# lukedan/libfluid

Hardware: AMD Instinct MI355X
Metric: particle_steps_per_sec (higher is better)
Workload: dtype f32

## Files before the change

libfluid_amd/csrc/particles.hip:

```cpp
#include <math.h>

#include <algorithm>
#include <utility>

#include "common.h"
#include "pcg.h"

namespace {

__device__ inline bool solid_or_outside(const GridDims &g, const uint8_t *solid, int x, int y, int z) {
	if (!in_grid(g, x, y, z)) return true;
	return solid[blocked_index(g, x, y, z)] != 0;
}

__device__ inline void collide(const GridDims &g, const uint8_t *solid, double from[3], double to[3], double skin) {
	for (int bounce = 0; bounce < 3; ++bounce) {
		bool hit = false;
		double diff[3], inv[3], t[3];
		int cur[3], last[3], adv[3];
#pragma unroll
		for (int d = 0; d < 3; ++d) {
			cur[d] = (int)floor(from[d]);
			last[d] = (int)floor(to[d]);
			diff[d] = to[d] - from[d];
// ... 60 lines not shown
		if (cp < skin && ci == 0) x += skin - cp;
		if (cp > skin_max && ci + 1 >= n[d]) x += skin_max - cp;
		to[d] = x;
	}
}

__device__ inline void cell_of_key(const GridDims &g, uint32_t key, int c[3]) {
	int tile = (int)(key >> 9), l = (int)(key & 511), tx, ty, tz;
	tile_coords(g, tile, tx, ty, tz);
	c[0] = tx * 8 + (l & 7); c[1] = ty * 8 + ((l >> 3) & 7); c[2] = tz * 8 + (l >> 6);
}
__device__ inline void split_position(double p, int n, int &cell, float &t) {
	double m = p < 0.0 ? 0.0 : p;
	int c = m >= (double)n ? n - 1 : (int)m;
	double td = p - (double)c;
	float tf = (float)td;
	if (!(tf > 0.0f)) tf = 0.0f;
	if (td < 1.0 && tf >= 1.0f) tf = 0.99999994f;
	if (tf > 1.0f) tf = 1.0f;
	cell = c;
	t = tf;
}

#ifndef CORR_PARTS
#define CORR_PARTS 2
#endif
#define CORR_THREADS 512
#define CORR_THREADS_BIG 1024
#ifndef CORR_STAGE_DEPTH
#define CORR_STAGE_DEPTH 4
#endif
#define CORR_BIG_SLICES 4

struct MoveParams {
	double dt_over_h;
	double skin;
	double corr;
	double inv_re2;
	float *c_home;
	size_t c_home_stride;
	int collide;
};

__global__ void __launch_bounds__(256) k_tile_has_solid(const uint8_t *solid, int nt, uint8_t *tile_solid) {
	for (int t = blockIdx.x; t < nt; t += gridDim.x) {
		const uint8_t *c = solid + (size_t)t * LFA_TILE_CELLS;
		const int any = __syncthreads_or((c[threadIdx.x] | c[threadIdx.x + 256]) != 0);
		if (threadIdx.x == 0) tile_solid[t] = (uint8_t)(any ? 1 : 0);
	}
}
__global__ void k_tile_clear(GridDims g, const uint8_t *tile_solid, uint8_t *tile_clear) {
	const int t = blockIdx.x * blockDim.x + threadIdx.x;
	if (t >= g.nt) return;
	int tx, ty, tz;
	tile_coords(g, t, tx, ty, tz);
	int any = 0;
	for (int dz = -1; dz <= 1; ++dz)
		for (int dy = -1; dy <= 1; ++dy)
			for (int dx = -1; dx <= 1; ++dx) {
				const int x = tx + dx, y = ty + dy, z = tz + dz;
				if ((unsigned)x < (unsigned)g.ntx && (unsigned)y < (unsigned)g.nty && (unsigned)z < (unsigned)g.ntz)
					any |= tile_solid[x + g.ntx * (y + g.nty * z)];
			}
	tile_clear[t] = (uint8_t)(any ? 0 : 1);
}

template <bool COERCE>
__device__ inline uint32_t advect_one(size_t i, const ParticleSoA &p, const GridDims &g, const uint8_t *solid, const MoveParams &mp,
                                      const uint8_t *coerce_map, const float *src_vel, const uint8_t *tile_clear) {
	const uint32_t key = p.key[i];
	if (key == 0xFFFFFFFFu) return key;
	int c[3];
	cell_of_key(g, key, c);
	const int nn[3] = {g.nx, g.ny, g.nz};
	float vel[3] = {p.v[0][i], p.v[1][i], p.v[2][i]};
	if (COERCE) {
		const uint32_t src = coerce_map[key];
		if (src) {
#pragma unroll
			for (int d = 0; d < 3; ++d) {
				vel[d] = src_vel[3 * (src - 1) + d];
				p.v[d][i] = vel[d];
			}
			if (mp.c_home) {
				const size_t j = p.id[i];
#pragma unroll
				for (int k = 0; k < 9; ++k) mp.c_home[k * mp.c_home_stride + j] = 0.0f;
			} else {
#pragma unroll
				for (int k = 0; k < 9; ++k) p.c[k][i] = 0.0f;
			}
		}
	}
	double from[3], to[3];
#pragma unroll
	for (int d = 0; d < 3; ++d) {
		from[d] = (double)c[d] + (double)p.t[d][i];
		double x = from[d] + (double)vel[d] * mp.dt_over_h;
		const double lo = mp.skin, hi = (double)nn[d] - mp.skin;
		to[d] = x < lo ? lo : (hi < x ? hi : x);
	}
	const bool open_water = (tile_clear[key >> 9] & 1) && fabs(to[0] - from[0]) < 7.0 && fabs(to[1] - from[1]) < 7.0 &&
	                        fabs(to[2] - from[2]) < 7.0;
	if (!open_water && mp.collide) collide(g, solid, from, to, mp.skin);
	int nc[3];
	float nt[3];
#pragma unroll
	for (int d = 0; d < 3; ++d) split_position(to[d], nn[d], nc[d], nt[d]);
	const uint32_t new_key = blocked_index(g, nc[0], nc[1], nc[2]);
	p.key[i] = new_key;
#pragma unroll
	for (int d = 0; d < 3; ++d) p.t[d][i] = nt[d];
	return new_key;
}

template <bool COERCE>
__global__ void __launch_bounds__(256)
k_advect_collide(size_t n, ParticleSoA p, GridDims g, const uint8_t *solid, MoveParams mp, const uint8_t *coerce_map,
                 const float *src_vel, const uint8_t *tile_clear) {
	const size_t i = (size_t)blockIdx.x * blockDim.x + threadIdx.x;
	if (i < n) advect_one<COERCE>(i, p, g, solid, mp, coerce_map, src_vel, tile_clear);
}

#define AC_CHUNKS 8
template <bool COERCE>
__global__ void __launch_bounds__(256)
k_advect_collide_count(size_t n, ParticleSoA p, GridDims g, const uint8_t *solid, MoveParams mp, const uint8_t *coerce_map,
                       const float *src_vel, const uint8_t *tile_clear, uint32_t *tile_count, uint32_t *rank) {
	const int lane = threadIdx.x & 63;
	const size_t wave = ((size_t)blockIdx.x * blockDim.x + threadIdx.x) >> 6;
	const size_t i0 = wave * (64 * AC_CHUNKS) + lane;
	uint32_t tile[AC_CHUNKS], my_rank[AC_CHUNKS];
#pragma unroll
	for (int c = 0; c < AC_CHUNKS; ++c) {
		const size_t i = i0 + 64 * c;
		const uint32_t k = i < n ? advect_one<COERCE>(i, p, g, solid, mp, coerce_map, src_vel, tile_clear) : 0xFFFFFFFFu;
		tile[c] = k != 0xFFFFFFFFu ? k >> 9 : 0xFFFFFFFFu;
	}
	lfa_wave_tile_ranks(tile, tile_count, my_rank);
#pragma unroll
	for (int c = 0; c < AC_CHUNKS; ++c) {
		const size_t i = i0 + 64 * c;
		if (tile[c] != 0xFFFFFFFFu) rank[i] = my_rank[c];
	}
}

__device__ inline float hash_unit(uint32_t a, uint32_t b, uint32_t k) {
	uint32_t x = a * 0x9E3779B1u ^ (b + 0x7F4A7C15u) * 0x85EBCA77u ^ k * 0xC2B2AE3Du;
	x ^= x >> 15; x *= 0x2C1B3C6Du; x ^= x >> 12; x *= 0x297A2D39u; x ^= x >> 15;
	return (float)(x >> 8) * (2.0f / 16777216.0f) - 1.0f;
}

#define FT 11
#define FT3 (FT * FT * FT)
#define FT_STRIDE (FT3 + 1)
#define FT_INV 1.375f
#define FT_PL ((FT + CORR_PARTS - 1) / CORR_PARTS)
#define FB 13
#define FBZ (FT_PL + 2)
#define FB_N (FB * FB * FBZ)
#define FB_ROWS (FB * FBZ)
#define FINE_CAP 5632
#define FINE_CAP_BIG 12288
#define FIDX_THREADS 512
#define FIDX_CNT 1536
#define FIDX_STAGE 4608

__device__ inline int fine_coord(int l, float t) {
	const int f = (int)(((float)l + t) * FT_INV);
	return f < FT - 1 ? f : FT - 1;
}
__device__ inline float4 fine_record(int lx, int ly, int lz, float t0, float t1, float t2, uint32_t index) {
	const uint32_t b0 = (__float_as_uint(t0) & 0x3FFFFFFFu) | ((uint32_t)(lx & 3) << 30);
	const uint32_t b1 = (__float_as_uint(t1) & 0x3FFFFFFFu) | ((uint32_t)(lx >> 2) << 31) | ((uint32_t)(ly & 1) << 30);
	const uint32_t b2 = (__float_as_uint(t2) & 0x3FFFFFFFu) | ((uint32_t)(lz & 1) << 31);
	return make_float4(__uint_as_float(b0), __uint_as_float(b1), __uint_as_float(b2), __uint_as_float(index));
}
__device__ inline void fine_decode_at(const float4 &r, int y0, int z0, float t[3], int l[3]) {
	const uint32_t b0 = __float_as_uint(r.x), b1 = __float_as_uint(r.y), b2 = __float_as_uint(r.z);
	t[0] = __uint_as_float(b0 & 0x3FFFFFFFu); t[1] = __uint_as_float(b1 & 0x3FFFFFFFu); t[2] = __uint_as_float(b2 & 0x3FFFFFFFu);
	l[0] = (int)(b0 >> 30) | ((int)(b1 >> 31) << 2);
	l[1] = y0 + ((y0 ^ (int)(b1 >> 30)) & 1);
	l[2] = z0 + ((z0 ^ (int)(b2 >> 31)) & 1);
}
__device__ inline void fine_decode(const float4 &r, int fy, int fz, float t[3], int l[3]) {
	fine_decode_at(r, (8 * fy) / FT, (8 * fz) / FT, t, l);
}

__global__ void __launch_bounds__(FIDX_THREADS)
k_build_fine_index(const int *ptiles, int n_ptiles, const uint32_t *key, const float *t0, const float *t1, const float *t2,
                   const uint32_t *tile_start, const uint32_t *tile_count, uint32_t *fine_start, float4 *spos, uint32_t *key_copy) {
	__shared__ uint32_t cnt[FIDX_CNT];
	__shared__ uint32_t wsum[FIDX_THREADS / 64];
	__shared__ float4 stage[FIDX_STAGE];
	static_assert(FIDX_CNT % FIDX_THREADS == 0 && FIDX_STAGE % FIDX_THREADS == 0, "index kernel sizing");
	constexpr int PER = FIDX_CNT / FIDX_THREADS;
	auto fine_of = [&](uint32_t i, int l[3], float t[3]) -> int {
		const uint32_t k = key[i];
		l[0] = (int)(k & 7); l[1] = (int)((k >> 3) & 7); l[2] = (int)((k >> 6) & 7);
		t[0] = t0[i]; t[1] = t1[i]; t[2] = t2[i];
		return fine_coord(l[0], t[0]) + FT * (fine_coord(l[1], t[1]) + FT * fine_coord(l[2], t[2]));
	};
	constexpr int RPT = FIDX_STAGE / FIDX_THREADS;
	for (int slot = blockIdx.x; slot < n_ptiles; slot += gridDim.x) {
		const int tile = ptiles[slot];
		const uint32_t b = tile_start[tile], e = b + tile_count[tile];
		const bool staged = e - b <= FIDX_STAGE;
#pragma unroll
		for (int k = 0; k < PER; ++k) cnt[threadIdx.x + FIDX_THREADS * k] = 0;
		__syncthreads();
		uint32_t rf[RPT];
		float r0[RPT], r1[RPT], r2[RPT];
		if (staged) {
#pragma unroll
			for (int r = 0; r < RPT; ++r) {
				const uint32_t i = b + threadIdx.x + FIDX_THREADS * r;
				rf[r] = 0xFFFFFFFFu;
				if (i < e) {
					int l[3];
					float t[3];
					const int f = fine_of(i, l, t);
					rf[r] = ((uint32_t)f << 9) | (uint32_t)(l[0] | (l[1] << 3) | (l[2] << 6));
					r0[r] = t[0]; r1[r] = t[1]; r2[r] = t[2];
					atomicAdd(&cnt[f], 1u);
				}
			}
		} else {
			for (uint32_t i = b + threadIdx.x; i < e; i += FIDX_THREADS) {
				int l[3];
				float t[3];
				atomicAdd(&cnt[fine_of(i, l, t)], 1u);
			}
		}
		__syncthreads();
		uint32_t c[PER], incl = 0;
#pragma unroll
		for (int k = 0; k < PER; ++k) {
			c[k] = cnt[PER * threadIdx.x + k];
			incl += c[k];
		}
		const uint32_t sum = incl;
		const int lane = threadIdx.x & 63, wid = threadIdx.x >> 6;
#pragma unroll
		for (int o = 1; o < 64; o <<= 1) {
			uint32_t t = __shfl_up(incl, o, 64);
			if (lane >= o) incl += t;
		}
		if (lane == 63) wsum[wid] = incl;
		__syncthreads();
		uint32_t ex = b + incl - sum;
		for (int w = 0; w < wid; ++w) ex += wsum[w];
		__syncthreads();
#pragma unroll
		for (int k = 0; k < PER; ++k) {
			const int f = PER * threadIdx.x + k;
			cnt[f] = ex;
			if (f <= FT3) fine_start[(size_t)tile * FT_STRIDE + f] = ex;
			ex += c[k];
		}
		__syncthreads();
		if (staged) {
#pragma unroll
			for (int r = 0; r < RPT; ++r)
				if (rf[r] != 0xFFFFFFFFu) {
					const uint32_t at = atomicAdd(&cnt[rf[r] >> 9], 1u);
					stage[at - b] = fine_record((int)(rf[r] & 7), (int)((rf[r] >> 3) & 7), (int)((rf[r] >> 6) & 7), r0[r], r1[r], r2[r],
					                            b + threadIdx.x + FIDX_THREADS * r);
				}
			if (key_copy) {
#pragma unroll
				for (int r = 0; r < RPT; ++r)
					if (rf[r] != 0xFFFFFFFFu) key_copy[b + threadIdx.x + FIDX_THREADS * r] = ((uint32_t)tile << 9) | (rf[r] & 511u);
			}
			__syncthreads();
			for (uint32_t k = threadIdx.x; k < e - b; k += FIDX_THREADS) spos[b + k] = stage[k];
		} else {
			for (uint32_t i = b + threadIdx.x; i < e; i += FIDX_THREADS) {
				int l[3];
				float t[3];
				const uint32_t at = atomicAdd(&cnt[fine_of(i, l, t)], 1u);
				spos[at] = fine_record(l[0], l[1], l[2], t[0], t[1], t[2], i);
				if (key_copy) key_copy[i] = key[i];
			}
		}
		__syncthreads();
	}
}

__device__ inline int fine_source(const GridDims &g, const uint32_t *tile_count, int tx, int ty, int tz, int gx, int gy, int gz, int &fx,
                                  int &fy, int &fz) {
	const int dx = gx < 0 ? -1 : (gx >= FT ? 1 : 0), dy = gy < 0 ? -1 : (gy >= FT ? 1 : 0), dz = gz < 0 ? -1 : (gz >= FT ? 1 : 0);
	fx = gx - FT * dx; fy = gy - FT * dy; fz = gz - FT * dz;
	const int x = tx + dx, y = ty + dy, z = tz + dz;
	if ((unsigned)x >= (unsigned)g.ntx || (unsigned)y >= (unsigned)g.nty || (unsigned)z >= (unsigned)g.ntz) return -1;
	const int tile = x + g.ntx * (y + g.nty * z);
	return tile_count[tile] ? tile : -1;
}

__device__ inline void correct_collide_record(size_t rk, const ParticleSoA &p, uint32_t *out_key, float *out_tx, float *out_ty, float *out_tz,
                                              const GridDims &g, const uint8_t *solid, const uint32_t *tile_count, const uint32_t *fine_start,
                                              const float4 *spos, const MoveParams &mp, const uint32_t *only_flagged, const int *tile_pslot,
                                              int p_off, const uint32_t *key_before) {
	const float4 me = spos[rk];
	const size_t i = __float_as_uint(me.w);
	const uint32_t key_i = key_before ? key_before[i] : p.key[i];
	if (key_i == 0xFFFFFFFFu) return;
	const int tile = (int)(key_i >> 9);
	const int l[3] = {(int)(key_i & 7), (int)((key_i >> 3) & 7), (int)((key_i >> 6) & 7)};
	const float t[3] = {__uint_as_float(__float_as_uint(me.x) & 0x3FFFFFFFu), __uint_as_float(__float_as_uint(me.y) & 0x3FFFFFFFu),
	                    __uint_as_float(__float_as_uint(me.z) & 0x3FFFFFFFu)};
	const int f[3] = {fine_coord(l[0], t[0]), fine_coord(l[1], t[1]), fine_coord(l[2], t[2])};
	if (only_flagged) {
		const int work = CORR_PARTS * (tile_pslot[tile] - p_off) + f[2] / FT_PL;
		if (!((only_flagged[1 + (work >> 5)] >> (work & 31)) & 1u)) return;
	}
	int tx, ty, tz;
	tile_coords(g, tile, tx, ty, tz);
	const int nn[3] = {g.nx, g.ny, g.nz};
	const float inv_re2 = (float)mp.inv_re2;
	double spring[3] = {0.0, 0.0, 0.0};
	for (int dz = -1; dz <= 1; ++dz)
		for (int dy = -1; dy <= 1; ++dy)
			for (int dx = -1; dx <= 1; ++dx) {
				int sf[3];
				const int src = fine_source(g, tile_count, tx, ty, tz, f[0] + dx, f[1] + dy, f[2] + dz, sf[0], sf[1], sf[2]);
				if (src < 0) continue;
				const uint32_t *fs = fine_start + (size_t)src * FT_STRIDE + (sf[0] + FT * (sf[1] + FT * sf[2]));
				const uint32_t kb = fs[0], ke = fs[1];
				int stx, sty, stz;
				tile_coords(g, src, stx, sty, stz);
				for (uint32_t k = kb; k < ke; ++k) {
					const float4 rec = spos[k];
					if (__float_as_uint(rec.w) == (uint32_t)i) continue;
					float nt[3];
					int nl[3];
					fine_decode(rec, sf[1], sf[2], nt, nl);
					const float ddx = ((float)(8 * (tx - stx) + l[0] - nl[0]) + t[0]) - nt[0];
					const float ddy = ((float)(8 * (ty - sty) + l[1] - nl[1]) + t[1]) - nt[1];
					const float ddz = ((float)(8 * (tz - stz) + l[2] - nl[2]) + t[2]) - nt[2];
					const float d2 = ddx * ddx + ddy * ddy + ddz * ddz;
					if (d2 < 1e-12f) {
						const uint32_t j = __float_as_uint(rec.w);
						spring[0] += hash_unit((uint32_t)i, j, 0); spring[1] += hash_unit((uint32_t)i, j, 1);
						spring[2] += hash_unit((uint32_t)i, j, 2);
					} else {
						const float kl = 1.0f - d2 * inv_re2;
						if (kl > 0.0f) {
							const float fr = kl * kl * kl * rsqrtf(d2);
							spring[0] += (double)(fr * ddx); spring[1] += (double)(fr * ddy); spring[2] += (double)(fr * ddz);
						}
					}
				}
			}
	const int c[3] = {8 * tx + l[0], 8 * ty + l[1], 8 * tz + l[2]};
	double from[3], to[3];
#pragma unroll
	for (int d = 0; d < 3; ++d) {
		from[d] = (double)c[d] + (double)t[d];
		double x = from[d] + spring[d] * mp.corr;
		to[d] = x < 0.0 ? 0.0 : ((double)nn[d] < x ? (double)nn[d] : x);
	}
	if (mp.collide) collide(g, solid, from, to, mp.skin);
	int nc[3];
	float ntt[3];
#pragma unroll
	for (int d = 0; d < 3; ++d) split_position(to[d], nn[d], nc[d], ntt[d]);
	out_key[i] = blocked_index(g, nc[0], nc[1], nc[2]);
	out_tx[i] = ntt[0]; out_ty[i] = ntt[1]; out_tz[i] = ntt[2];
}

__global__ void __launch_bounds__(256)
k_correct_collide(size_t n, ParticleSoA p, uint32_t *out_key, float *out_tx, float *out_ty, float *out_tz, GridDims g,
                   const uint8_t *solid, const uint32_t *tile_count, const uint32_t *fine_start, const float4 *spos, MoveParams mp,
                   const uint32_t *only_flagged, const int *tile_pslot, int p_off, const uint32_t *key_before) {
	if (only_flagged && only_flagged[0] == 0) return;
	for (size_t rk = (size_t)blockIdx.x * blockDim.x + threadIdx.x; rk < n; rk += (size_t)gridDim.x * blockDim.x)
		correct_collide_record(rk, p, out_key, out_tx, out_ty, out_tz, g, solid, tile_count, fine_start, spos, mp, only_flagged, tile_pslot,
		                       p_off, key_before);
}

#ifdef CORR_PROFILE
__device__ unsigned long long g_corr_prof[8];
#define CORR_STAMP(k)                                                                   \
	do {                                                                                \
		if (!ONLY && threadIdx.x == 0) {                                                \
			const unsigned long long now_ = wall_clock64();                             \
			atomicAdd(&g_corr_prof[k], now_ - stamp_);                                  \
			stamp_ = now_;                                                              \
		}                                                                               \
	} while (0)
#else
#define CORR_STAMP(k) do { } while (0)
#endif
template <int CAP, bool ONLY>
__global__ void __launch_bounds__(ONLY ? CORR_THREADS_BIG : CORR_THREADS, 4)
k_correct_fine(const int *ptiles, int n_ptiles, uint32_t *out_key, float *out_tx, float *out_ty, float *out_tz, GridDims g,
                const uint8_t *solid, const uint32_t *tile_count, const uint32_t *fine_start, const float4 *spos, MoveParams mp,
                uint32_t *overflow_tiles, const uint8_t *tile_clear, const uint32_t *only) {
	constexpr int T = ONLY ? CORR_THREADS_BIG : CORR_THREADS;
	constexpr int CNT = ((FB_N + 1 + T - 1) / T) * T;
	__shared__ float px[CAP], py[CAP], pz[CAP];
	__shared__ uint32_t fcnt[CNT];
	__shared__ uint16_t foff[FB_N + 1];
	__shared__ __attribute__((aligned(16))) uint32_t rowd[FB_ROWS * 8];
	constexpr uint32_t ROW_NOT_OWN = 0x80000000u;
	__shared__ uint32_t ownoff[FT * FT_PL + 1];
	__shared__ int srct[27];
	__shared__ uint32_t wsum[T / 64];
	uint16_t *own = (uint16_t *)fcnt;
	static_assert(CNT > FB_N && CNT % T == 0, "fcnt sizing");
	constexpr int PER = CNT / T;
	const int nn[3] = {g.nx, g.ny, g.nz};
	const int lane = threadIdx.x & 63, wid = threadIdx.x >> 6;
	if (ONLY && only[0] == 0) return;
	constexpr int SLICES = ONLY ? CORR_BIG_SLICES : 1;
	for (int item = blockIdx.x; item < SLICES * CORR_PARTS * n_ptiles; item += gridDim.x) {
		const int work = item / SLICES, slice = item % SLICES;
		if (ONLY && !((only[1 + (work >> 5)] >> (work & 31)) & 1u)) continue;
		const int tile = ptiles[work / CORR_PARTS], part = work % CORR_PARTS;
		int tx, ty, tz;
		tile_coords(g, tile, tx, ty, tz);
		const int own_lo = part * FT_PL, own_n = (own_lo + FT_PL <= FT ? FT_PL : FT - own_lo);
		const int gz0 = own_lo - 1;
		const int nzb = own_n + 2;
		const int nrows = FB * nzb, nown_rows = FT * (nzb - 2);
		const bool open_water = (tile_clear[tile] & 1) != 0;
		const bool lean = open_water && mp.collide && tx >= 1 && ty >= 1 && tz >= 1 && 8 * tx + 16 <= g.nx && 8 * ty + 16 <= g.ny &&
		                  8 * tz + 16 <= g.nz;
		__syncthreads();
#ifdef CORR_PROFILE
		unsigned long long stamp_ = wall_clock64();
		if (!ONLY && threadIdx.x == 0) atomicAdd(&g_corr_prof[7], 1ull);
#endif
		uint32_t tid = threadIdx.x;
		asm volatile("" : "+v"(tid));
		if (tid < 27) {
			int fx, fy, fz;
			srct[tid] = fine_source(g, tile_count, tx, ty, tz, FT * ((int)tid % 3 - 1), FT * (((int)tid / 3) % 3 - 1), FT * ((int)tid / 9 - 1), fx,
			                        fy, fz);
		}
		__syncthreads();
#pragma unroll
		for (int k = 0; k < PER; ++k) {
			const int f = (int)(k == PER - 1 ? tid : threadIdx.x) + T * k;
			uint32_t cnt = 0, src0 = 0;
			if (f < FB * nrows) {
				const int bx = f % FB, row = f / FB, by = row % FB, bz = row / FB;
				const int gx = bx - 1, gy = by - 1, gz = gz0 + bz;
				const int dx = gx < 0 ? 0 : (gx >= FT ? 2 : 1), dy = gy < 0 ? 0 : (gy >= FT ? 2 : 1), dz = gz < 0 ? 0 : (gz >= FT ? 2 : 1);
				const int src = srct[dx + 3 * dy + 9 * dz];
				if (src >= 0) {
					const uint32_t fid = (uint32_t)((gx - FT * (dx - 1)) + FT * ((gy - FT * (dy - 1)) + FT * (gz - FT * (dz - 1))));
					const uint32_t *fs = fine_start + ((uint32_t)src * FT_STRIDE + fid);
					src0 = fs[0];
					cnt = fs[1] - src0;
				}
				if (bx <= 1 || bx == FB - 1) rowd[row * 8 + (bx <= 1 ? bx : 2)] = src0;
			}
			fcnt[f] = cnt;
		}
		__syncthreads();
		uint32_t c4[PER], sum = 0;
#pragma unroll
		for (int k = 0; k < PER; ++k) {
			c4[k] = fcnt[PER * threadIdx.x + k];
			sum += c4[k];
		}
		uint32_t incl = sum;
#pragma unroll
		for (int o = 1; o < 64; o <<= 1) {
			uint32_t t = __shfl_up(incl, o, 64);
			if (lane >= o) incl += t;
		}
		if (lane == 63) wsum[wid] = incl;
		__syncthreads();
		uint32_t woff = 0, total = 0;
		for (int w = 0; w < T / 64; ++w) {
			if (w < wid) woff += wsum[w];
			total += wsum[w];
		}
		if (total > (uint32_t)CAP) {
			if (threadIdx.x == 0 && slice == 0) {
				atomicOr(&overflow_tiles[1 + (work >> 5)], 1u << (work & 31));
				atomicAdd(&overflow_tiles[0], 1u);
			}
			continue;
		}
		{
			uint32_t ex = woff + incl - sum;
#pragma unroll
			for (int k = 0; k < PER; ++k) {
				const int f = PER * threadIdx.x + k;
				if (f <= FB_N) foff[f] = (uint16_t)ex;
				ex += c4[k];
			}
		}
		__syncthreads();
		uint32_t own_total = 0, own_first = 0;
		{
			uint32_t len = 0;
			if (tid < (unsigned)nown_rows) {
				const int row = (1 + (int)tid % FT) + FB * (1 + (int)tid / FT);
				len = (uint32_t)foff[row * FB + FB - 1] - (uint32_t)foff[row * FB + 1];
			}
			uint32_t in2 = len;
#pragma unroll
			for (int o = 1; o < 64; o <<= 1) {
				uint32_t t = __shfl_up(in2, o, 64);
				if (lane >= o) in2 += t;
			}
			if (lane == 63) wsum[wid] = in2;
			__syncthreads();
			uint32_t wo = 0;
			for (int w = 0; w < T / 64; ++w) {
				if (w < wid) wo += wsum[w];
				own_total += wsum[w];
			}
			own_first = wo + in2 - len;
			if (tid < (unsigned)nown_rows) ownoff[tid] = own_first;
			if (tid == 0) ownoff[nown_rows] = own_total;
		}
		const bool listed = own_total <= 2u * CNT;
		if (tid < (unsigned)nrows) {
			const int r = (int)tid, by = r % FB, bz = r / FB;
			const int gy = by - 1, gz = gz0 + bz;
			const int dy = gy < 0 ? -1 : (gy >= FT ? 1 : 0), dz = gz < 0 ? -1 : (gz >= FT ? 1 : 0);
			const int fy = gy - FT * dy, fz = gz - FT * dz;
			const uint32_t d0 = foff[r * FB], d1 = foff[r * FB + 1], d2 = foff[r * FB + FB - 1];
			uint32_t *rd = rowd + r * 8;
			rd[0] -= d0; rd[1] -= d1; rd[2] -= d2;
			rd[3] = d1 | (d2 << 16);
			rd[4] = (uint32_t)(8 * dy); rd[5] = (uint32_t)(8 * dz);
			rd[6] = (uint32_t)((8 * fy) / FT) | ((uint32_t)((8 * fz) / FT) << 8);
			if (!(listed && by >= 1 && by <= FT && bz >= 1 && bz <= nzb - 2)) rd[7] = ROW_NOT_OWN;
		}
		if (listed && tid < (unsigned)nown_rows) {
			const int row = (1 + (int)tid % FT) + FB * (1 + (int)tid / FT);
			rowd[row * 8 + 7] = own_first - (uint32_t)foff[row * FB + 1];
		}
		__syncthreads();
		CORR_STAMP(0);
		{
			static_assert(FB_ROWS <= 128, "two row starts per lane");
			const int rl = (int)(tid & 63u);
			const uint32_t rs_lo = rl < nrows ? (uint32_t)foff[rl * FB] : 0xFFFFFFFFu;
			const uint32_t rs_hi = rl + 64 < nrows ? (uint32_t)foff[(rl + 64) * FB] : 0xFFFFFFFFu;
			auto row_of = [&](uint32_t s) -> int {
				return (int)__popcll(__ballot(rs_lo <= s)) + (int)__popcll(__ballot(rs_hi <= s)) - 1;
			};
			auto locate = [&](uint32_t slot, int r_first, int r_last, uint32_t &src, int &rs) {
				int r = r_first;
				const int span = r_last - r_first;
				for (int step = span ? 1 << (31 - __builtin_clz(span)) : 0; step; step >>= 1) {
					const int c = r + step;
					if (c <= r_last && (uint32_t)foff[c * FB] <= slot) r = c;
				}
				const uint4 d = *(const uint4 *)(rowd + r * 8);
				const int seg = slot < (d.w & 0xFFFFu) ? 0 : (slot < (d.w >> 16) ? 1 : 2);
				src = (seg == 0 ? d.x : (seg == 1 ? d.y : d.z)) + slot;
				rs = r | (seg << 8);
			};
			auto put = [&](uint32_t slot, const float4 &rec, int rs) {
				const int r = rs & 255, seg = rs >> 8;
				const uint4 d = *(const uint4 *)(rowd + r * 8 + 4);
				float t[3];
				int l[3];
				fine_decode_at(rec, (int)(d.z & 255u), (int)(d.z >> 8), t, l);
				px[slot] = (float)(8 * (seg - 1) + l[0]) + t[0];
				py[slot] = (float)((int)d.x + l[1]) + t[1];
				pz[slot] = (float)((int)d.y + l[2]) + t[2];
				if (seg == 1 && d.w != ROW_NOT_OWN) own[d.w + slot] = (uint16_t)slot;
			};
			const uint32_t wave0 = (uint32_t)__builtin_amdgcn_readfirstlane((int)(threadIdx.x & ~63u));
			for (uint32_t w0 = wave0; w0 < total; w0 += CORR_STAGE_DEPTH * T) {
				uint32_t src[CORR_STAGE_DEPTH];
				int rs[CORR_STAGE_DEPTH];
				float4 rec[CORR_STAGE_DEPTH];
#pragma unroll
				for (int u = 0; u < CORR_STAGE_DEPTH; ++u) {
					const uint32_t wu = w0 + u * T, slot = wu + lane;
					src[u] = 0; rs[u] = 0;
					if (wu < total) {
						const uint32_t last = wu + 63 < total ? wu + 63 : total - 1;
						const int r_first = row_of(wu), r_last = row_of(last);
						if (slot < total) locate(slot, r_first, r_last, src[u], rs[u]);
					}
				}
#pragma unroll
				for (int u = 0; u < CORR_STAGE_DEPTH; ++u) rec[u] = spos[src[u]];
#pragma unroll
				for (int u = 0; u < CORR_STAGE_DEPTH; ++u) {
					const uint32_t slot = w0 + u * T + lane;
					if (slot < total) put(slot, rec[u], rs[u]);
				}
			}
		}
		__syncthreads();
		CORR_STAMP(1);
#ifdef CORR_PROFILE
		if (!ONLY && threadIdx.x == 0) { atomicAdd(&g_corr_prof[5], (unsigned long long)total); atomicAdd(&g_corr_prof[6], (unsigned long long)own_total); }
#endif
		for (uint32_t w = threadIdx.x + T * slice; w < own_total; w += T * SLICES) {
			uint32_t me;
			if (listed) {
				me = own[w];
			} else {
				int lo = 0, hi = nown_rows - 1;
				while (lo < hi) {
					const int mid = (lo + hi + 1) >> 1;
					if (ownoff[mid] <= w) lo = mid;
					else hi = mid - 1;
				}
				me = (uint32_t)foff[((1 + lo % FT) + FB * (1 + lo / FT)) * FB + 1] + (w - ownoff[lo]);
			}
#ifdef CORR_PROFILE
			const unsigned long long w0_ = wall_clock64();
#endif
			const float mx = px[me], my = py[me], mz = pz[me];
			int fx = (int)(mx * FT_INV), fy = (int)(my * FT_INV), fz = (int)(mz * FT_INV);
			fx = fx < FT - 1 ? fx : FT - 1; fy = fy < FT - 1 ? fy : FT - 1; fz = fz < FT - 1 ? fz : FT - 1;
			const int bx = fx + 1, by = fy + 1, bz = fz - gz0;
			float sx = 0.f, sy = 0.f, sz = 0.f;
			typedef float f2 __attribute__((ext_vector_type(2)));
			f2 s2x = 0.f, s2y = 0.f, s2z = 0.f;
			const float inv_re2 = (float)mp.inv_re2;
			uint32_t j = 0xFFFFFFFFu;
			const uint32_t myrow = by + FB * bz;
			const uint32_t grec = rowd[myrow * 8 + 1] + me;
			auto pair2 = [&](uint32_t q, f2 qx, f2 qy, f2 qz) {
				const f2 dx = mx - qx, dy = my - qy, dz = mz - qz;
				const f2 d2 = __builtin_elementwise_fma(dz, dz, __builtin_elementwise_fma(dy, dy, dx * dx));
				const f2 kl = __builtin_elementwise_fma(-d2, (f2)inv_re2, (f2)1.0f);
				if (kl.x > 0.0f || kl.y > 0.0f) {
#pragma unroll
					for (int k = 0; k < 2; ++k) {
						const float d2k = k ? d2.y : d2.x, klk = k ? kl.y : kl.x;
						if (!(klk > 0.0f)) continue;
						if (d2k < 1e-12f) {
							if (q + k != me) {
								if (j == 0xFFFFFFFFu) j = __float_as_uint(spos[grec].w);
								sx += hash_unit(j, q + k, 0); sy += hash_unit(j, q + k, 1); sz += hash_unit(j, q + k, 2);
							}
						} else {
							const float f = klk * klk * klk * rsqrtf(d2k);
							sx += f * (k ? dx.y : dx.x); sy += f * (k ? dy.y : dy.x); sz += f * (k ? dz.y : dz.x);
						}
					}
				}
			};
			auto walk = [&](auto &&p2, auto &&p2_centre) {
				for (int dz = -1; dz <= 1; ++dz)
					for (int dy = -1; dy <= 1; ++dy) {
						const int rowf = FB * ((by + dy) + FB * (bz + dz)) + bx;
						const uint32_t b = foff[rowf - 1], e = foff[rowf + 2];
						auto run = [&](auto &&pp) {
							uint32_t q = b;
							for (; q + 4 <= e; q += 4) {
								const float x0 = px[q], x1 = px[q + 1], x2 = px[q + 2], x3 = px[q + 3];
								const float y0 = py[q], y1 = py[q + 1], y2 = py[q + 2], y3 = py[q + 3];
								const float z0 = pz[q], z1 = pz[q + 1], z2 = pz[q + 2], z3 = pz[q + 3];
								pp(q, f2{x0, x1}, f2{y0, y1}, f2{z0, z1});
								pp(q + 2, f2{x2, x3}, f2{y2, y3}, f2{z2, z3});
							}
							if (q + 2 <= e) {
								pp(q, f2{px[q], px[q + 1]}, f2{py[q], py[q + 1]}, f2{pz[q], pz[q + 1]});
								q += 2;
							}
							if (q < e) pp(q, f2{px[q], 1e6f}, f2{py[q], 1e6f}, f2{pz[q], 1e6f});
						};
						if (dy == 0 && dz == 0) run(p2_centre);
						else run(p2);
					}
			};
			float d2_min = 1.0f;
			uint32_t n_tiny = 0;
			auto fast = [&](f2 qx, f2 qy, f2 qz) -> f2 {
				const f2 dx = mx - qx, dy = my - qy, dz = mz - qz;
				const f2 d2 = __builtin_elementwise_fma(dz, dz, __builtin_elementwise_fma(dy, dy, __builtin_elementwise_fma(dx, dx, (f2)1e-30f)));
				f2 kl;
				kl.x = __builtin_amdgcn_fmed3f(__builtin_fmaf(-d2.x, inv_re2, 1.0f), 0.0f, 1.0f);
				kl.y = __builtin_amdgcn_fmed3f(__builtin_fmaf(-d2.y, inv_re2, 1.0f), 0.0f, 1.0f);
				f2 f = kl * kl * kl;
				f.x *= __builtin_amdgcn_rsqf(d2.x);
				f.y *= __builtin_amdgcn_rsqf(d2.y);
				s2x = __builtin_elementwise_fma(f, dx, s2x);
				s2y = __builtin_elementwise_fma(f, dy, s2y);
				s2z = __builtin_elementwise_fma(f, dz, s2z);
				return d2;
			};
			walk([&](uint32_t, f2 qx, f2 qy, f2 qz) {
					     const f2 d2 = fast(qx, qy, qz);
					     d2_min = fminf(d2_min, fminf(d2.x, d2.y));
				     },
				     [&](uint32_t, f2 qx, f2 qy, f2 qz) {
					     const f2 d2 = fast(qx, qy, qz);
					     n_tiny += (d2.x < 1e-12f ? 1u : 0u) + (d2.y < 1e-12f ? 1u : 0u);
				     });
			if (d2_min < 1e-12f || n_tiny != 1u) {
				s2x = 0.f; s2y = 0.f; s2z = 0.f;
				walk(pair2, pair2);
			}
			sx += s2x.x + s2x.y;
			sy += s2y.x + s2y.y;
			sz += s2z.x + s2z.y;
#ifdef CORR_PROFILE
			if (!ONLY && threadIdx.x == 0) atomicAdd(&g_corr_prof[4], wall_clock64() - w0_);
#endif
			float tme[3];
			int lme[3];
			const float4 rec = spos[grec];
			const uint32_t yz = rowd[myrow * 8 + 6];
			fine_decode_at(rec, (int)(yz & 255u), (int)(yz >> 8), tme, lme);
			const uint32_t jj = __float_as_uint(rec.w);
			const int c[3] = {8 * tx + lme[0], 8 * ty + lme[1], 8 * tz + lme[2]};
			const double spring[3] = {(double)sx, (double)sy, (double)sz};
			double from[3], to[3];
#pragma unroll
			for (int d = 0; d < 3; ++d) {
				from[d] = (double)c[d] + (double)tme[d];
				to[d] = from[d] + spring[d] * mp.corr;
			}
			if (!(lean && fabs(to[0] - from[0]) < 7.0 && fabs(to[1] - from[1]) < 7.0 && fabs(to[2] - from[2]) < 7.0)) {
#pragma unroll
				for (int d = 0; d < 3; ++d) to[d] = to[d] < 0.0 ? 0.0 : ((double)nn[d] < to[d] ? (double)nn[d] : to[d]);
				if (mp.collide) {
					if (!open_water || fabs(to[0] - from[0]) >= 7.0 || fabs(to[1] - from[1]) >= 7.0 || fabs(to[2] - from[2]) >= 7.0)
						collide(g, solid, from, to, mp.skin);
					else
						collide_walls_only(g, to, mp.skin);
				}
			}
			int nc[3];
			float nt[3];
#pragma unroll
			for (int d = 0; d < 3; ++d) split_position(to[d], nn[d], nc[d], nt[d]);
			out_key[jj] = blocked_index(g, nc[0], nc[1], nc[2]);
			out_tx[jj] = nt[0]; out_ty[jj] = nt[1]; out_tz[jj] = nt[2];
		}
#ifdef CORR_PROFILE
		CORR_STAMP(2);
		__syncthreads();
		CORR_STAMP(3);
#endif
	}
}

}
#ifdef CORR_PROFILE
extern "C" int lfa_debug_corr_prof(uint64_t out[8], int reset) {
	unsigned long long h[8] = {0};
	if (hipMemcpyFromSymbol(h, HIP_SYMBOL(g_corr_prof), sizeof h) != hipSuccess) return -1;
	for (int i = 0; i < 8; ++i) out[i] = h[i];
	if (reset) {
		unsigned long long z[8] = {0};
		if (hipMemcpyToSymbol(HIP_SYMBOL(g_corr_prof), z, sizeof z) != hipSuccess) return -1;
	}
	return 0;
}
#endif

static MoveParams move_params(const lfa_sim *s, double dt) {
	MoveParams mp;
	const double h = s->prm.cell_size, re = h / sqrt(2.0);
	mp.dt_over_h = dt / h;
	mp.skin = s->prm.boundary_skin_width / h;
	mp.corr = dt * s->prm.correction_stiffness * re / h;
	mp.inv_re2 = h * h / (re * re);
	mp.collide = 1;
	mp.c_home = s->c_home_valid ? s->c_home : nullptr;
	mp.c_home_stride = s->c_home_cap;
	return mp;
}


namespace {
__global__ void k_mark_coerce(const uint32_t *cell, const uint32_t *src1, size_t n, uint8_t *map) {
	const size_t i = (size_t)blockIdx.x * blockDim.x + threadIdx.x;
	if (i < n) map[cell[i]] = (uint8_t)src1[i];
}
__global__ void k_source_need(const uint32_t *cell, const uint32_t *lo, const uint32_t *target, size_t n, const uint32_t *cell_count,
                              const uint32_t *tile_flag, uint32_t *need) {
	const size_t i = (size_t)blockIdx.x * blockDim.x + threadIdx.x;
	if (i >= n) return;
	const uint32_t b = cell[i];
	const uint32_t have = lo[i] != 0xFFFFFFFFu ? lo[i] : (tile_flag[b >> 9] ? cell_count[b] : 0u);
	need[i] = target[i] > have ? target[i] - have : 0u;
}
__global__ void k_source_need_scatter(const uint32_t *need, const uint32_t *gidx, size_t n, float *all) {
	const size_t i = (size_t)blockIdx.x * blockDim.x + threadIdx.x;
	if (i < n) all[gidx[i]] = (float)need[i];
}
__global__ void k_source_need_gather(const float *all, size_t n, uint32_t *need) {
	const size_t i = (size_t)blockIdx.x * blockDim.x + threadIdx.x;
	if (i < n) need[i] = (uint32_t)all[i];
}
__device__ inline uint64_t mix64(uint64_t x) {
	x ^= x >> 30; x *= 0xBF58476D1CE4E5B9ull;
	x ^= x >> 27; x *= 0x94D049BB133111EBull;
	x ^= x >> 31;
	return x;
}
__global__ void k_source_seed(const uint32_t *cell, const uint32_t *src_of, const uint32_t *need, const uint32_t *off, size_t n,
                              const float *src_vel, ParticleSoA p, size_t base, uint64_t seed, uint64_t id_base) {
	const size_t i = (size_t)blockIdx.x * blockDim.x + threadIdx.x;
	if (i >= n) return;
	const uint32_t cnt = need[i], b = cell[i];
	const float *vel = src_vel + 3 * src_of[i];
	for (uint32_t j = 0; j < cnt; ++j) {
		const size_t d = base + off[i] + j;
		p.key[d] = b;
#pragma unroll
		for (int a = 0; a < 3; ++a) {
			const uint64_t r = mix64(seed + ((id_base + (uint64_t)(d - base)) * 3ull + (uint64_t)a + 1ull) * 0x9E3779B97F4A7C15ull + ((uint64_t)b << 40));
			float t = (float)(r >> 40) * (1.0f / 16777216.0f);
			p.t[a][d] = t;
			p.v[a][d] = vel[a];
		}
		particle_zero_c_set_id(p, d, (uint32_t)(id_base + (uint64_t)(d - base)));
	}
}
}

extern "C" int lfa_clear_sources(lfa_sim *s) {
	if (!s) return LFA_E_INVALID;
	s->sources.clear();
	s->sources_valid = false;
	return LFA_OK;
}

extern "C" int lfa_add_source(lfa_sim *s, const int32_t *xyz, uint64_t k, const double velocity[3], uint64_t root, int active,
                              int coerce_velocity) {
	if (!s || (!xyz && k) || !velocity) return LFA_E_INVALID;
	if (s->sources.size() >= 254) return lfa_fail(s, LFA_E_UNSUPPORTED, "more than 254 fluid sources");
	if (root > 16) return lfa_fail(s, LFA_E_INVALID, "target_density_cubic_root %llu: more than 4096 particles per cell", (unsigned long long)root);
	for (uint64_t i = 0; i < k; ++i)
		if (!in_grid(s->g, xyz[3 * i], xyz[3 * i + 1], xyz[3 * i + 2]))
			return lfa_fail(s, LFA_E_INVALID, "source cell (%d, %d, %d) outside the grid", xyz[3 * i], xyz[3 * i + 1], xyz[3 * i + 2]);
	lfa_sim::SourceHost h;
	h.xyz.assign(xyz, xyz + 3 * k);
	for (int d = 0; d < 3; ++d) h.vel[d] = velocity[d];
	h.root = root;
	h.active = active != 0;
	h.coerce = coerce_velocity != 0;
	s->sources.push_back(std::move(h));
	s->sources_valid = false;
	return LFA_OK;
}

int lfa_sources_sync(lfa_sim *s) {
	if (s->sources_valid) return LFA_OK;
	if (s->sources == s->sources_built && (s->sources.empty() || s->src_vel)) {
		s->sources_valid = true;
		return LFA_OK;
	}
	LFA_HIP(s, hipSetDevice(s->device));
	const int own_zlo = s->dist ? s->slab_lo * 8 : 0, own_zhi = s->dist ? s->slab_hi * 8 : s->g.nz;
	std::vector<uint32_t> cell, lo, target, of, ccell, csrc;
	std::vector<uint32_t> own_g, k_cell, k_of, k_g, k_mode;
	uint32_t n_global = 0;
	std::vector<float> vel;
	{
		std::vector<std::pair<uint32_t, uint32_t>> seen;
		std::vector<std::pair<uint32_t, uint32_t>> coerce;
		for (size_t si = 0; si < s->sources.size(); ++si) {
			const auto &h = s->sources[si];
// ... 704 lines not shown
```

Baseline: 5.031 billion.

## Halve fine-cell width along x and pack shared-memory counters into 16-bit halves

Splits each tile's fine neighbour grid into twice as many cells along x (22 instead of 11), so the correction kernel's neighbour walk scans a 5-cell window of narrower cells rather than 3 wider ones. The intent is fewer candidate pairs per particle in the spring/correction loop. Counters in the index builder and the correction kernel are packed two per 32-bit word as 16-bit values, and the per-row metadata is compressed into a smaller rowd plus a packed rowe word, to keep shared memory use in check. The costs are more fine-index entries to build and read, more range lookups per walk, and 16-bit count limits that clamp at 0xFFFF.

```diff
diff --git a/libfluid_amd/csrc/particles.hip b/libfluid_amd/csrc/particles.hip
--- a/libfluid_amd/csrc/particles.hip
+++ b/libfluid_amd/csrc/particles.hip
@@ -236,23 +236,30 @@
 }
 
 #define FT 11
-#define FT3 (FT * FT * FT)
+#define FTX (2 * FT)
+#define FT3 (FTX * FT * FT)
 #define FT_STRIDE (FT3 + 1)
 #define FT_INV 1.375f
+#define FTX_INV 2.75f
 #define FT_PL ((FT + CORR_PARTS - 1) / CORR_PARTS)
 #define FB 13
+#define FBX (FTX + 4)
 #define FBZ (FT_PL + 2)
-#define FB_N (FB * FB * FBZ)
+#define FB_N (FBX * FB * FBZ)
 #define FB_ROWS (FB * FBZ)
 #define FINE_CAP 5632
 #define FINE_CAP_BIG 12288
 #define FIDX_THREADS 512
-#define FIDX_CNT 1536
+#define FIDX_CNT (((FT3 + 1 + FIDX_THREADS - 1) / FIDX_THREADS) * FIDX_THREADS)
 #define FIDX_STAGE 4608
 
 __device__ inline int fine_coord(int l, float t) {
 	const int f = (int)(((float)l + t) * FT_INV);
 	return f < FT - 1 ? f : FT - 1;
+}
+__device__ inline int fine_coord_x(int l, float t) {
+	const int f = (int)(((float)l + t) * FTX_INV);
+	return f < FTX - 1 ? f : FTX - 1;
 }
 __device__ inline float4 fine_record(int lx, int ly, int lz, float t0, float t1, float t2, uint32_t index) {
 	const uint32_t b0 = (__float_as_uint(t0) & 0x3FFFFFFFu) | ((uint32_t)(lx & 3) << 30);
@@ -274,24 +281,31 @@
 __global__ void __launch_bounds__(FIDX_THREADS)
 k_build_fine_index(const int *ptiles, int n_ptiles, const uint32_t *key, const float *t0, const float *t1, const float *t2,
                    const uint32_t *tile_start, const uint32_t *tile_count, uint32_t *fine_start, float4 *spos, uint32_t *key_copy) {
-	__shared__ uint32_t cnt[FIDX_CNT];
+	__shared__ uint32_t cnt[FIDX_CNT / 2];
 	__shared__ uint32_t wsum[FIDX_THREADS / 64];
 	__shared__ float4 stage[FIDX_STAGE];
-	static_assert(FIDX_CNT % FIDX_THREADS == 0 && FIDX_STAGE % FIDX_THREADS == 0, "index kernel sizing");
+	static_assert(FIDX_CNT % (2 * FIDX_THREADS) == 0 && FIDX_STAGE % FIDX_THREADS == 0 && FIDX_STAGE < 65536 && FIDX_CNT <= 4 * FIDX_STAGE,
+	              "index kernel sizing");
 	constexpr int PER = FIDX_CNT / FIDX_THREADS;
+	uint32_t *cnt_big = (uint32_t *)stage;
 	auto fine_of = [&](uint32_t i, int l[3], float t[3]) -> int {
 		const uint32_t k = key[i];
 		l[0] = (int)(k & 7); l[1] = (int)((k >> 3) & 7); l[2] = (int)((k >> 6) & 7);
 		t[0] = t0[i]; t[1] = t1[i]; t[2] = t2[i];
-		return fine_coord(l[0], t[0]) + FT * (fine_coord(l[1], t[1]) + FT * fine_coord(l[2], t[2]));
+		return fine_coord_x(l[0], t[0]) + FTX * (fine_coord(l[1], t[1]) + FT * fine_coord(l[2], t[2]));
 	};
 	constexpr int RPT = FIDX_STAGE / FIDX_THREADS;
 	for (int slot = blockIdx.x; slot < n_ptiles; slot += gridDim.x) {
 		const int tile = ptiles[slot];
 		const uint32_t b = tile_start[tile], e = b + tile_count[tile];
 		const bool staged = e - b <= FIDX_STAGE;
-#pragma unroll
-		for (int k = 0; k < PER; ++k) cnt[threadIdx.x + FIDX_THREADS * k] = 0;
+		if (staged) {
+#pragma unroll
+			for (int k = 0; k < PER / 2; ++k) cnt[threadIdx.x + FIDX_THREADS * k] = 0;
+		} else {
+#pragma unroll
+			for (int k = 0; k < PER; ++k) cnt_big[threadIdx.x + FIDX_THREADS * k] = 0;
+		}
 		__syncthreads();
 		uint32_t rf[RPT];
 		float r0[RPT], r1[RPT], r2[RPT];
@@ -306,21 +320,21 @@
 					const int f = fine_of(i, l, t);
 					rf[r] = ((uint32_t)f << 9) | (uint32_t)(l[0] | (l[1] << 3) | (l[2] << 6));
 					r0[r] = t[0]; r1[r] = t[1]; r2[r] = t[2];
-					atomicAdd(&cnt[f], 1u);
+					atomicAdd(&cnt[f >> 1], 1u << (16 * (f & 1)));
 				}
 			}
 		} else {
 			for (uint32_t i = b + threadIdx.x; i < e; i += FIDX_THREADS) {
 				int l[3];
 				float t[3];
-				atomicAdd(&cnt[fine_of(i, l, t)], 1u);
+				atomicAdd(&cnt_big[fine_of(i, l, t)], 1u);
 			}
 		}
 		__syncthreads();
 		uint32_t c[PER], incl = 0;
 #pragma unroll
 		for (int k = 0; k < PER; ++k) {
-			c[k] = cnt[PER * threadIdx.x + k];
+			c[k] = staged ? (cnt[(PER / 2) * threadIdx.x + k / 2] >> (16 * (k & 1))) & 0xFFFFu : cnt_big[PER * threadIdx.x + k];
 			incl += c[k];
 		}
 		const uint32_t sum = incl;
@@ -332,14 +346,15 @@
 		}
 		if (lane == 63) wsum[wid] = incl;
 		__syncthreads();
-		uint32_t ex = b + incl - sum;
+		uint32_t ex = incl - sum;
 		for (int w = 0; w < wid; ++w) ex += wsum[w];
 		__syncthreads();
 #pragma unroll
 		for (int k = 0; k < PER; ++k) {
 			const int f = PER * threadIdx.x + k;
-			cnt[f] = ex;
-			if (f <= FT3) fine_start[(size_t)tile * FT_STRIDE + f] = ex;
+			if (!staged) cnt_big[f] = ex;
+			else if (k & 1) cnt[f >> 1] = (ex - c[k - (k & 1)]) | (ex << 16);
+			if (!staged && f <= FT3) fine_start[(size_t)tile * FT_STRIDE + f] = b + ex;
 			ex += c[k];
 		}
 		__syncthreads();
@@ -347,9 +362,10 @@
 #pragma unroll
 			for (int r = 0; r < RPT; ++r)
 				if (rf[r] != 0xFFFFFFFFu) {
-					const uint32_t at = atomicAdd(&cnt[rf[r] >> 9], 1u);
-					stage[at - b] = fine_record((int)(rf[r] & 7), (int)((rf[r] >> 3) & 7), (int)((rf[r] >> 6) & 7), r0[r], r1[r], r2[r],
-					                            b + threadIdx.x + FIDX_THREADS * r);
+					const uint32_t f = rf[r] >> 9;
+					const uint32_t at = (atomicAdd(&cnt[f >> 1], 1u << (16 * (f & 1))) >> (16 * (f & 1))) & 0xFFFFu;
+					stage[at] = fine_record((int)(rf[r] & 7), (int)((rf[r] >> 3) & 7), (int)((rf[r] >> 6) & 7), r0[r], r1[r], r2[r],
+					                        b + threadIdx.x + FIDX_THREADS * r);
 				}
 			if (key_copy) {
 #pragma unroll
@@ -357,13 +373,15 @@
 					if (rf[r] != 0xFFFFFFFFu) key_copy[b + threadIdx.x + FIDX_THREADS * r] = ((uint32_t)tile << 9) | (rf[r] & 511u);
 			}
 			__syncthreads();
+			for (int f = threadIdx.x; f <= FT3; f += FIDX_THREADS)
+				fine_start[(size_t)tile * FT_STRIDE + f] = b + (f ? (cnt[(f - 1) >> 1] >> (16 * ((f - 1) & 1))) & 0xFFFFu : 0u);
 			for (uint32_t k = threadIdx.x; k < e - b; k += FIDX_THREADS) spos[b + k] = stage[k];
 		} else {
 			for (uint32_t i = b + threadIdx.x; i < e; i += FIDX_THREADS) {
 				int l[3];
 				float t[3];
-				const uint32_t at = atomicAdd(&cnt[fine_of(i, l, t)], 1u);
-				spos[at] = fine_record(l[0], l[1], l[2], t[0], t[1], t[2], i);
+				const uint32_t at = atomicAdd(&cnt_big[fine_of(i, l, t)], 1u);
+				spos[b + at] = fine_record(l[0], l[1], l[2], t[0], t[1], t[2], i);
 				if (key_copy) key_copy[i] = key[i];
 			}
 		}
@@ -373,8 +391,8 @@
 
 __device__ inline int fine_source(const GridDims &g, const uint32_t *tile_count, int tx, int ty, int tz, int gx, int gy, int gz, int &fx,
                                   int &fy, int &fz) {
-	const int dx = gx < 0 ? -1 : (gx >= FT ? 1 : 0), dy = gy < 0 ? -1 : (gy >= FT ? 1 : 0), dz = gz < 0 ? -1 : (gz >= FT ? 1 : 0);
-	fx = gx - FT * dx; fy = gy - FT * dy; fz = gz - FT * dz;
+	const int dx = gx < 0 ? -1 : (gx >= FTX ? 1 : 0), dy = gy < 0 ? -1 : (gy >= FT ? 1 : 0), dz = gz < 0 ? -1 : (gz >= FT ? 1 : 0);
+	fx = gx - FTX * dx; fy = gy - FT * dy; fz = gz - FT * dz;
 	const int x = tx + dx, y = ty + dy, z = tz + dz;
 	if ((unsigned)x >= (unsigned)g.ntx || (unsigned)y >= (unsigned)g.nty || (unsigned)z >= (unsigned)g.ntz) return -1;
 	const int tile = x + g.ntx * (y + g.nty * z);
@@ -393,7 +411,7 @@
 	const int l[3] = {(int)(key_i & 7), (int)((key_i >> 3) & 7), (int)((key_i >> 6) & 7)};
 	const float t[3] = {__uint_as_float(__float_as_uint(me.x) & 0x3FFFFFFFu), __uint_as_float(__float_as_uint(me.y) & 0x3FFFFFFFu),
 	                    __uint_as_float(__float_as_uint(me.z) & 0x3FFFFFFFu)};
-	const int f[3] = {fine_coord(l[0], t[0]), fine_coord(l[1], t[1]), fine_coord(l[2], t[2])};
+	const int f[3] = {fine_coord_x(l[0], t[0]), fine_coord(l[1], t[1]), fine_coord(l[2], t[2])};
 	if (only_flagged) {
 		const int work = CORR_PARTS * (tile_pslot[tile] - p_off) + f[2] / FT_PL;
 		if (!((only_flagged[1 + (work >> 5)] >> (work & 31)) & 1u)) return;
@@ -405,11 +423,11 @@
 	double spring[3] = {0.0, 0.0, 0.0};
 	for (int dz = -1; dz <= 1; ++dz)
 		for (int dy = -1; dy <= 1; ++dy)
-			for (int dx = -1; dx <= 1; ++dx) {
+			for (int dx = -2; dx <= 2; ++dx) {
 				int sf[3];
 				const int src = fine_source(g, tile_count, tx, ty, tz, f[0] + dx, f[1] + dy, f[2] + dz, sf[0], sf[1], sf[2]);
 				if (src < 0) continue;
-				const uint32_t *fs = fine_start + (size_t)src * FT_STRIDE + (sf[0] + FT * (sf[1] + FT * sf[2]));
+				const uint32_t *fs = fine_start + (size_t)src * FT_STRIDE + (sf[0] + FTX * (sf[1] + FT * sf[2]));
 				const uint32_t kb = fs[0], ke = fs[1];
 				int stx, sty, stz;
 				tile_coords(g, src, stx, sty, stz);
@@ -482,17 +500,20 @@
                 const uint8_t *solid, const uint32_t *tile_count, const uint32_t *fine_start, const float4 *spos, MoveParams mp,
                 uint32_t *overflow_tiles, const uint8_t *tile_clear, const uint32_t *only) {
 	constexpr int T = ONLY ? CORR_THREADS_BIG : CORR_THREADS;
-	constexpr int CNT = ((FB_N + 1 + T - 1) / T) * T;
+	constexpr int CNT0 = ((FB_N + 1 + 2 * T - 1) / (2 * T)) * (2 * T);
+	constexpr int CNT = ONLY && CNT0 < 4096 ? 4096 : CNT0;
 	__shared__ float px[CAP], py[CAP], pz[CAP];
-	__shared__ uint32_t fcnt[CNT];
+	__shared__ uint32_t fcnt2[CNT / 2];
+	uint16_t *fcnt = (uint16_t *)fcnt2;
 	__shared__ uint16_t foff[FB_N + 1];
-	__shared__ __attribute__((aligned(16))) uint32_t rowd[FB_ROWS * 8];
-	constexpr uint32_t ROW_NOT_OWN = 0x80000000u;
+	__shared__ __attribute__((aligned(16))) uint32_t rowd[FB_ROWS * 4];
+	__shared__ uint32_t rowe[FB_ROWS];
+	constexpr int ROW_NOT_OWN = -32768;
 	__shared__ uint32_t ownoff[FT * FT_PL + 1];
 	__shared__ int srct[27];
 	__shared__ uint32_t wsum[T / 64];
-	uint16_t *own = (uint16_t *)fcnt;
-	static_assert(CNT > FB_N && CNT % T == 0, "fcnt sizing");
+	uint16_t *own = fcnt;
+	static_assert(CNT > FB_N && CNT % (2 * T) == 0 && FBX % 2 == 0 && CAP < 32768 && CNT < 32768, "fcnt sizing");
 	constexpr int PER = CNT / T;
 	const int nn[3] = {g.nx, g.ny, g.nz};
 	const int lane = threadIdx.x & 63, wid = threadIdx.x >> 6;
@@ -520,28 +541,31 @@
 		asm volatile("" : "+v"(tid));
 		if (tid < 27) {
 			int fx, fy, fz;
-			srct[tid] = fine_source(g, tile_count, tx, ty, tz, FT * ((int)tid % 3 - 1), FT * (((int)tid / 3) % 3 - 1), FT * ((int)tid / 9 - 1), fx,
+			srct[tid] = fine_source(g, tile_count, tx, ty, tz, FTX * ((int)tid % 3 - 1), FT * (((int)tid / 3) % 3 - 1), FT * ((int)tid / 9 - 1), fx,
 			                        fy, fz);
 		}
 		__syncthreads();
-#pragma unroll
-		for (int k = 0; k < PER; ++k) {
-			const int f = (int)(k == PER - 1 ? tid : threadIdx.x) + T * k;
-			uint32_t cnt = 0, src0 = 0;
-			if (f < FB * nrows) {
-				const int bx = f % FB, row = f / FB, by = row % FB, bz = row / FB;
-				const int gx = bx - 1, gy = by - 1, gz = gz0 + bz;
-				const int dx = gx < 0 ? 0 : (gx >= FT ? 2 : 1), dy = gy < 0 ? 0 : (gy >= FT ? 2 : 1), dz = gz < 0 ? 0 : (gz >= FT ? 2 : 1);
+		constexpr int ROUNDS = CNT / (2 * T), KEPT = ROUNDS - 1 < 2 ? ROUNDS - 1 : 2;
+#pragma unroll
+		for (int k = 0; k < ROUNDS; ++k) {
+			const int p = (int)(k >= KEPT ? tid : threadIdx.x) + T * k;
+			uint32_t cnt0 = 0, cnt1 = 0, src0 = 0;
+			if (p < (FBX / 2) * nrows) {
+				const int bx = 2 * (p % (FBX / 2)), row = p / (FBX / 2), by = row % FB, bz = row / FB;
+				const int gx = bx - 2, gy = by - 1, gz = gz0 + bz;
+				const int dx = gx < 0 ? 0 : (gx >= FTX ? 2 : 1), dy = gy < 0 ? 0 : (gy >= FT ? 2 : 1), dz = gz < 0 ? 0 : (gz >= FT ? 2 : 1);
 				const int src = srct[dx + 3 * dy + 9 * dz];
 				if (src >= 0) {
-					const uint32_t fid = (uint32_t)((gx - FT * (dx - 1)) + FT * ((gy - FT * (dy - 1)) + FT * (gz - FT * (dz - 1))));
+					const uint32_t fid = (uint32_t)((gx - FTX * (dx - 1)) + FTX * ((gy - FT * (dy - 1)) + FT * (gz - FT * (dz - 1))));
 					const uint32_t *fs = fine_start + ((uint32_t)src * FT_STRIDE + fid);
 					src0 = fs[0];
-					cnt = fs[1] - src0;
+					const uint32_t mid = fs[1];
+					cnt0 = mid - src0;
+					cnt1 = fs[2] - mid;
 				}
-				if (bx <= 1 || bx == FB - 1) rowd[row * 8 + (bx <= 1 ? bx : 2)] = src0;
-			}
-			fcnt[f] = cnt;
+				if (bx == 0 || bx == 2 || bx == FBX - 2) rowd[row * 4 + (bx == 0 ? 0 : (bx == 2 ? 1 : 2))] = src0;
+			}
+			fcnt2[p] = (cnt0 < 0xFFFFu ? cnt0 : 0xFFFFu) | ((cnt1 < 0xFFFFu ? cnt1 : 0xFFFFu) << 16);
 		}
 		__syncthreads();
 		uint32_t c4[PER], sum = 0;
@@ -585,7 +609,7 @@
 			uint32_t len = 0;
 			if (tid < (unsigned)nown_rows) {
 				const int row = (1 + (int)tid % FT) + FB * (1 + (int)tid / FT);
-				len = (uint32_t)foff[row * FB + FB - 1] - (uint32_t)foff[row * FB + 1];
+				len = (uint32_t)foff[row * FBX + FBX - 2] - (uint32_t)foff[row * FBX + 2];
 			}
 			uint32_t in2 = len;
 #pragma unroll
@@ -604,31 +628,31 @@
 			if (tid < (unsigned)nown_rows) ownoff[tid] = own_first;
 			if (tid == 0) ownoff[nown_rows] = own_total;
 		}
-		const bool listed = own_total <= 2u * CNT;
+		const bool listed = own_total <= (uint32_t)CNT;
 		if (tid < (unsigned)nrows) {
 			const int r = (int)tid, by = r % FB, bz = r / FB;
 			const int gy = by - 1, gz = gz0 + bz;
 			const int dy = gy < 0 ? -1 : (gy >= FT ? 1 : 0), dz = gz < 0 ? -1 : (gz >= FT ? 1 : 0);
 			const int fy = gy - FT * dy, fz = gz - FT * dz;
-			const uint32_t d0 = foff[r * FB], d1 = foff[r * FB + 1], d2 = foff[r * FB + FB - 1];
-			uint32_t *rd = rowd + r * 8;
+			const uint32_t d0 = foff[r * FBX], d1 = foff[r * FBX + 2], d2 = foff[r * FBX + FBX - 2];
+			uint32_t *rd = rowd + r * 4;
 			rd[0] -= d0; rd[1] -= d1; rd[2] -= d2;
 			rd[3] = d1 | (d2 << 16);
-			rd[4] = (uint32_t)(8 * dy); rd[5] = (uint32_t)(8 * dz);
-			rd[6] = (uint32_t)((8 * fy) / FT) | ((uint32_t)((8 * fz) / FT) << 8);
-			if (!(listed && by >= 1 && by <= FT && bz >= 1 && bz <= nzb - 2)) rd[7] = ROW_NOT_OWN;
-		}
+			rowe[r] = (uint32_t)((8 * fy) / FT) | ((uint32_t)((8 * fz) / FT) << 3) | ((uint32_t)(8 * (dy + 1)) << 6) |
+			          ((uint32_t)(8 * (dz + 1)) << 11) | ((uint32_t)ROW_NOT_OWN << 16);
+		}
+		__syncthreads();
 		if (listed && tid < (unsigned)nown_rows) {
 			const int row = (1 + (int)tid % FT) + FB * (1 + (int)tid / FT);
-			rowd[row * 8 + 7] = own_first - (uint32_t)foff[row * FB + 1];
+			rowe[row] = (rowe[row] & 0xFFFFu) | ((own_first - (uint32_t)foff[row * FBX + 2]) << 16);
 		}
 		__syncthreads();
 		CORR_STAMP(0);
 		{
 			static_assert(FB_ROWS <= 128, "two row starts per lane");
 			const int rl = (int)(tid & 63u);
-			const uint32_t rs_lo = rl < nrows ? (uint32_t)foff[rl * FB] : 0xFFFFFFFFu;
-			const uint32_t rs_hi = rl + 64 < nrows ? (uint32_t)foff[(rl + 64) * FB] : 0xFFFFFFFFu;
+			const uint32_t rs_lo = rl < nrows ? (uint32_t)foff[rl * FBX] : 0xFFFFFFFFu;
+			const uint32_t rs_hi = rl + 64 < nrows ? (uint32_t)foff[(rl + 64) * FBX] : 0xFFFFFFFFu;
 			auto row_of = [&](uint32_t s) -> int {
 				return (int)__popcll(__ballot(rs_lo <= s)) + (int)__popcll(__ballot(rs_hi <= s)) - 1;
 			};
@@ -637,23 +661,24 @@
 				const int span = r_last - r_first;
 				for (int step = span ? 1 << (31 - __builtin_clz(span)) : 0; step; step >>= 1) {
 					const int c = r + step;
-					if (c <= r_last && (uint32_t)foff[c * FB] <= slot) r = c;
+					if (c <= r_last && (uint32_t)foff[c * FBX] <= slot) r = c;
 				}
-				const uint4 d = *(const uint4 *)(rowd + r * 8);
+				const uint4 d = *(const uint4 *)(rowd + r * 4);
 				const int seg = slot < (d.w & 0xFFFFu) ? 0 : (slot < (d.w >> 16) ? 1 : 2);
 				src = (seg == 0 ? d.x : (seg == 1 ? d.y : d.z)) + slot;
 				rs = r | (seg << 8);
 			};
 			auto put = [&](uint32_t slot, const float4 &rec, int rs) {
 				const int r = rs & 255, seg = rs >> 8;
-				const uint4 d = *(const uint4 *)(rowd + r * 8 + 4);
+				const uint32_t d = rowe[r];
+				const int ob = (int)d >> 16;
 				float t[3];
 				int l[3];
-				fine_decode_at(rec, (int)(d.z & 255u), (int)(d.z >> 8), t, l);
+				fine_decode_at(rec, (int)(d & 7u), (int)((d >> 3) & 7u), t, l);
 				px[slot] = (float)(8 * (seg - 1) + l[0]) + t[0];
-				py[slot] = (float)((int)d.x + l[1]) + t[1];
-				pz[slot] = (float)((int)d.y + l[2]) + t[2];
-				if (seg == 1 && d.w != ROW_NOT_OWN) own[d.w + slot] = (uint16_t)slot;
+				py[slot] = (float)((int)((d >> 6) & 31u) - 8 + l[1]) + t[1];
+				pz[slot] = (float)((int)((d >> 11) & 31u) - 8 + l[2]) + t[2];
+				if (seg == 1 && ob != ROW_NOT_OWN) own[ob + (int)slot] = (uint16_t)slot;
 			};
 			const uint32_t wave0 = (uint32_t)__builtin_amdgcn_readfirstlane((int)(threadIdx.x & ~63u));
 			for (uint32_t w0 = wave0; w0 < total; w0 += CORR_STAGE_DEPTH * T) {
@@ -695,22 +720,22 @@
 					if (ownoff[mid] <= w) lo = mid;
 					else hi = mid - 1;
 				}
-				me = (uint32_t)foff[((1 + lo % FT) + FB * (1 + lo / FT)) * FB + 1] + (w - ownoff[lo]);
+				me = (uint32_t)foff[((1 + lo % FT) + FB * (1 + lo / FT)) * FBX + 2] + (w - ownoff[lo]);
 			}
 #ifdef CORR_PROFILE
 			const unsigned long long w0_ = wall_clock64();
 #endif
 			const float mx = px[me], my = py[me], mz = pz[me];
-			int fx = (int)(mx * FT_INV), fy = (int)(my * FT_INV), fz = (int)(mz * FT_INV);
-			fx = fx < FT - 1 ? fx : FT - 1; fy = fy < FT - 1 ? fy : FT - 1; fz = fz < FT - 1 ? fz : FT - 1;
-			const int bx = fx + 1, by = fy + 1, bz = fz - gz0;
+			int fx = (int)(mx * FTX_INV), fy = (int)(my * FT_INV), fz = (int)(mz * FT_INV);
+			fx = fx < FTX - 1 ? fx : FTX - 1; fy = fy < FT - 1 ? fy : FT - 1; fz = fz < FT - 1 ? fz : FT - 1;
+			const int bx = fx + 2, by = fy + 1, bz = fz - gz0;
 			float sx = 0.f, sy = 0.f, sz = 0.f;
 			typedef float f2 __attribute__((ext_vector_type(2)));
 			f2 s2x = 0.f, s2y = 0.f, s2z = 0.f;
 			const float inv_re2 = (float)mp.inv_re2;
 			uint32_t j = 0xFFFFFFFFu;
 			const uint32_t myrow = by + FB * bz;
-			const uint32_t grec = rowd[myrow * 8 + 1] + me;
+			const uint32_t grec = rowd[myrow * 4 + 1] + me;
 			auto pair2 = [&](uint32_t q, f2 qx, f2 qy, f2 qz) {
 				const f2 dx = mx - qx, dy = my - qy, dz = mz - qz;
 				const f2 d2 = __builtin_elementwise_fma(dz, dz, __builtin_elementwise_fma(dy, dy, dx * dx));
@@ -735,8 +760,8 @@
 			auto walk = [&](auto &&p2, auto &&p2_centre) {
 				for (int dz = -1; dz <= 1; ++dz)
 					for (int dy = -1; dy <= 1; ++dy) {
-						const int rowf = FB * ((by + dy) + FB * (bz + dz)) + bx;
-						const uint32_t b = foff[rowf - 1], e = foff[rowf + 2];
+						const int rowf = FBX * ((by + dy) + FB * (bz + dz)) + bx;
+						const uint32_t b = foff[rowf - 2], e = foff[rowf + 3];
 						auto run = [&](auto &&pp) {
 							uint32_t q = b;
 							for (; q + 4 <= e; q += 4) {
@@ -793,8 +818,8 @@
 			float tme[3];
 			int lme[3];
 			const float4 rec = spos[grec];
-			const uint32_t yz = rowd[myrow * 8 + 6];
-			fine_decode_at(rec, (int)(yz & 255u), (int)(yz >> 8), tme, lme);
+			const uint32_t yz = rowe[myrow];
+			fine_decode_at(rec, (int)(yz & 7u), (int)((yz >> 3) & 7u), tme, lme);
 			const uint32_t jj = __float_as_uint(rec.w);
 			const int c[3] = {8 * tx + lme[0], 8 * ty + lme[1], 8 * tz + lme[2]};
 			const double spring[3] = {(double)sx, (double)sy, (double)sz};
```

Result: faster. 5.165 billion, median of 6 (+2.7%).
